# factoryofthesun/distraytracer

Hardware: AMD Instinct MI355X
Metric: Mpixel-samples/s (W×H×spp/s) + wall-clock per frame, 1/2/4/8 GPU (higher is better)
Workload: dtype f64; 1 GPU; buildFinal(240) 1920x1080, 64 spp, depth 8, brdf_samples 2, DoF aperture 0.2, glossy + Cook-Torrance + 4 area lights; use_model=0, frame=240, xRes=1920, yRes=1080, spp=64, max_depth=8, parallelism=single GPU, 2 frame(s) in flight

## Files before the change

distraytracer_amd/__init__.py:

```python
import ctypes

from ._lib import (DATA_DIR, DT_KERNEL_AUTO, DT_KERNEL_DONATE, DT_KERNEL_PRODUCT, DT_OUT_IMAGE, DT_OUT_SLAB, AccelInfo, BVHNode, Camera, DenoiseParams, DenoiseVarParams, DTError, Globals, SceneDesc,
                   SHAPE_TYPES, OcclusionParams, RayOrderParams, DT_RAY_ORDER_TILE, Stats, TemporalParams, Tiles, UpsampleParams, check, lib)

__all__ = ["Globals", "Tiles", "Stats", "DTError", "globals_default", "build_scene", "Scene",
           "render", "render_sky", "renderImage", "renderImageCloud", "write_ppm", "DATA_DIR",
           "DT_OUT_IMAGE", "DT_OUT_SLAB", "slab_floats", "slab_floats_max", "unpack_slabs", "tiles", "check", "lib",
           "accel_info", "DT_KERNEL_AUTO", "DT_KERNEL_PRODUCT", "DT_KERNEL_DONATE",
           "accum_doubles", "window_check", "render_window", "render_window_async", "resolve", "Progressive",
           "mean_abs_change", "adapt_converged", "render_window_adaptive", "resolve_adaptive", "adapt_select_ms",
           "AdaptiveProgressive", "render_features", "feature_images", "FEATURE_PLANES",
           "DenoiseParams", "denoise_params_default", "denoise", "denoised_filename",
           "DenoiseVarParams", "denoise_var_params_default", "variance",
           "Camera", "camera", "TemporalParams", "temporal_params_default", "reproject", "TemporalAccumulator",
           "trace_rays", "rays_occluded", "RAY_PLANES",
           "trace_rays_multi", "segment_through_glass", "RAY_MULTI_PLANES",
           "rays_transmittance", "RAY_TRANSMIT_PLANES",
           "camera_rays", "camera_rays_rows", "rays_resolve", "peel_layers", "RESOLVE_MODES",
           "RayOrderParams", "RayOrder", "ray_order_params_default", "ray_order_key", "ray_order", "DT_RAY_ORDER_TILE",
           "render_mattes", "matte_mask", "shape_groups", "MATTE_PLANES",
           "UpsampleParams", "upsample_params_default", "upsample", "low_res_globals",
           "OcclusionParams", "occlusion_params_default", "render_occlusion", "occlusion_ao_ray", "occlusion_light_ray",
           "occlusion_images", "points_occlusion", "shape_texels", "bake_occlusion"]


def globals_default():
    g = Globals()
    lib.dt_globals_default(ctypes.byref(g))
    return g


# ... 8 lines not shown

    @property
    def desc(self):
        return self._ptr.contents

    def __del__(self):
        if getattr(self, "_ptr", None) and lib is not None:
            lib.dt_scene_desc_free(self._ptr)
            self._ptr = None


def build_scene(name, frame, g, data_dir=DATA_DIR):
    out = ctypes.POINTER(SceneDesc)()
    check(lib.dt_build_scene(name.encode(), float(frame), ctypes.byref(g), data_dir.encode(), ctypes.byref(out)),
          "dt_build_scene(%s)" % name)
    return BuiltScene(out)


def accel_info(built, g):
    info = AccelInfo()
    desc = built._ptr if isinstance(built, BuiltScene) else ctypes.pointer(built)
    check(lib.dt_accel_info_build(desc, ctypes.byref(g), ctypes.byref(info)), "dt_accel_info_build")
    return info.as_dict()


def trace_build(built, g, frame):
    name = ctypes.create_string_buffer(64)
    sf, bf = ctypes.c_uint32(), ctypes.c_uint32()
    desc = built._ptr if isinstance(built, BuiltScene) else ctypes.pointer(built)
    check(lib.dt_trace_build(desc, ctypes.byref(g), int(frame), name, 64, ctypes.byref(sf), ctypes.byref(bf)),
          "dt_trace_build")
    return name.value.decode(), sf.value, bf.value


class Scene:

    def __init__(self, built, g, upload=True):
        self._h = ctypes.c_void_p()
        desc = built._ptr if isinstance(built, BuiltScene) else ctypes.pointer(built)
        self._keep = built
        if upload:
            check(lib.dt_scene_create(desc, ctypes.byref(g), ctypes.byref(self._h)), "dt_scene_create")
        else:
            check(lib.dt_scene_prepare(desc, ctypes.byref(g), ctypes.byref(self._h)), "dt_scene_prepare")

    def upload(self):
# ... 1548 lines not shown
```

distraytracer_amd/_lib.py:

```python
import ctypes
import os

_HERE = os.path.dirname(os.path.abspath(__file__))
LIB_PATH = os.environ.get("DT_LIB") or os.path.join(_HERE, "libdt.so")
REPO_ROOT = os.path.dirname(_HERE)
DATA_DIR = os.path.join(REPO_ROOT, "data")

c_int32, c_uint32, c_int64, c_uint64 = ctypes.c_int32, ctypes.c_uint32, ctypes.c_int64, ctypes.c_uint64
c_float, c_double = ctypes.c_float, ctypes.c_double
D3 = c_double * 3

DT_OK = 0
DT_OUT_IMAGE = 0
DT_OUT_SLAB = 1
DT_KERNEL_AUTO, DT_KERNEL_PRODUCT, DT_KERNEL_DONATE = 0, 1, 2

SHAPE_TYPES = {1: "sphere", 2: "cylinder", 3: "triangle", 4: "rectangle", 5: "rectprism_v2",
               6: "checkerboard", 7: "checkerboard_hole", 8: "checker_cylinder", 9: "rectprism_cyl"}
ABI_VERSION = 8


class ShapeDesc(ctypes.Structure):
    _fields_ = [("type", c_int32), ("model", c_int32), ("material", c_int32), ("emit", c_int32),
                ("flags", c_uint32), ("tex_frame", c_int32), ("roughness", c_float), ("radius", c_float),
# ... 146 lines not shown

class History(ctypes.Structure):
    _fields_ = [("colour", ctypes.c_void_p), ("var", ctypes.c_void_p), ("len", ctypes.c_void_p)]


class BVHNode(ctypes.Structure):
    _fields_ = [("first_child", c_int32), ("n_children", c_int32), ("first_index", c_int32),
                ("n_indices", c_int32), ("leaf", c_int32), ("depth", c_int32), ("lbound", D3), ("ubound", D3)]


class AccelInfo(ctypes.Structure):
    _fields_ = [("n_nodes", c_int32), ("n_fnodes", c_int32), ("n_bnodes", c_int32), ("boxes_ordered", c_int32),
                ("sg_lights", c_int32), ("sg_dim", c_int32 * 3), ("sg_cells", c_int64), ("sg_tree_cells", c_int64),
                ("sg_list_pool", c_int64), ("sg_list_entries", c_int64), ("nodes_hash", c_uint64),
                ("fnodes_hash", c_uint64), ("bnodes_hash", c_uint64), ("sg_hash", c_uint64),
                ("sg_contents_hash", c_uint64), ("bump_pad", c_float), ("sg_reach", c_float),
                ("sg_umbra_cells", c_int64), ("features", ctypes.c_uint32),
                ("sg_sub_blocks", c_int32), ("sg_sub_nodes", c_int64), ("sg_sub_hash", c_uint64)]

    def as_dict(self):
        d = {k: getattr(self, k) for k, _ in self._fields_}
        d["sg_dim"] = tuple(self.sg_dim)
        return d


EXPORTS = ["dt_abi_version", "dt_last_error", "dt_globals_default", "dt_scene_create", "dt_scene_destroy",
           "dt_scene_prepare", "dt_scene_upload", "dt_scene_set_kernel",
           "dt_scene_bvh", "dt_bvh_build", "dt_accel_info_build", "dt_trace_build", "dt_slab_floats", "dt_slab_floats_max",
           "dt_render", "dt_render_async", "dt_collect_stats", "dt_debug_counters", "dt_debug_item_costs", "dt_render_sky",
           "dt_unpack_slabs", "dt_build_scene", "dt_scene_desc_free", "dt_write_ppm", "dt_write_png",
           "dt_mocap_bone_table", "dt_debug_normalize", "dt_debug_vdiv", "dt_debug_vnorm", "dt_debug_light_edges",
           "dt_intersect_primary",
           "dt_debug_load_obj",
           "dt_accum_doubles", "dt_window_check", "dt_render_window", "dt_render_window_async", "dt_resolve",
           "dt_adapt_converged", "dt_render_window_adaptive", "dt_render_window_adaptive_async",
           "dt_resolve_adaptive", "dt_adapt_select_ms", "dt_render_features",
           "dt_denoise_params_default", "dt_denoise_workspace_floats", "dt_denoise",
           "dt_variance", "dt_denoise_var_params_default", "dt_denoise_var_workspace_floats", "dt_denoise_var",
           "dt_camera_get", "dt_temporal_params_default", "dt_reproject",
           "dt_trace_rays", "dt_rays_occluded", "dt_render_mattes", "dt_matte_mask",
           "dt_upsample_params_default", "dt_upsample",
           "dt_guide_bounce", "dt_render_features_path",
           "dt_occlusion_params_default", "dt_render_occlusion", "dt_occlusion_ao_ray", "dt_occlusion_light_ray",
           "dt_points_occlusion",
           "dt_ray_order_params_default", "dt_ray_order_key", "dt_ray_order_workspace_bytes", "dt_ray_order",
           "dt_permute_rows",
           "dt_trace_rays_multi",
           "dt_camera_rays_rows", "dt_camera_rays", "dt_rays_resolve",
           "dt_rays_transmittance", "dt_points_occlusion_glass"]


class DTError(RuntimeError):
    pass


def _share_torch_hip_runtime():
    try:
        import torch
    except ImportError:
        pass


def _load():
    _share_torch_hip_runtime()
    if not os.path.exists(LIB_PATH):
        raise DTError("libdt.so not built (%s): run __graft_entry__.build() / make -C "
                      "distraytracer_amd/csrc" % LIB_PATH)
    lib = ctypes.CDLL(LIB_PATH)
    lib.dt_abi_version.restype = c_int32
    if lib.dt_abi_version() != ABI_VERSION:
        raise DTError("libdt.so ABI %d, this binding expects %d: rebuild (make -C distraytracer_amd/csrc)"
                      % (lib.dt_abi_version(), ABI_VERSION))
    P = ctypes.POINTER
    sig = {
        "dt_abi_version": (c_int32, []),
        "dt_last_error": (ctypes.c_char_p, []),
        "dt_globals_default": (None, [P(Globals)]),
        "dt_scene_create": (c_int32, [P(SceneDesc), P(Globals), P(ctypes.c_void_p)]),
        "dt_scene_destroy": (None, [ctypes.c_void_p]),
        "dt_scene_prepare": (c_int32, [P(SceneDesc), P(Globals), P(ctypes.c_void_p)]),
        "dt_scene_upload": (c_int32, [ctypes.c_void_p]),
        "dt_scene_set_kernel": (c_int32, [ctypes.c_void_p, c_int32]),
        "dt_scene_bvh": (c_int32, [ctypes.c_void_p, P(BVHNode), c_int32, P(c_int32), c_int32, P(c_int32),
                                   P(c_int32)]),
        "dt_bvh_build": (c_int32, [P(SceneDesc), P(Globals), P(BVHNode), c_int32, P(c_int32), c_int32, P(c_int32),
                                   P(c_int32)]),
        "dt_accel_info_build": (c_int32, [P(SceneDesc), P(Globals), P(AccelInfo)]),
        "dt_trace_build": (c_int32, [P(SceneDesc), P(Globals), c_int32, ctypes.c_char_p, c_int32,
                                     P(ctypes.c_uint32), P(ctypes.c_uint32)]),
        "dt_slab_floats": (c_int64, [P(Globals), P(Tiles)]),
        "dt_slab_floats_max": (c_int64, [P(Globals), P(Tiles)]),
        "dt_render": (c_int32, [ctypes.c_void_p, P(Globals), c_int32, P(Tiles), ctypes.c_void_p, c_int32,
                                ctypes.c_void_p, P(Stats)]),
        "dt_render_async": (c_int32, [ctypes.c_void_p, P(Globals), c_int32, P(Tiles), ctypes.c_void_p,
                                      ctypes.c_void_p]),
        "dt_collect_stats": (c_int32, [ctypes.c_void_p, ctypes.c_void_p, P(Stats)]),
        "dt_accum_doubles": (c_int64, [P(Globals), P(Tiles)]),
        "dt_window_check": (c_int32, [P(Globals), c_int32, c_int32]),
        "dt_render_window": (c_int32, [ctypes.c_void_p, P(Globals), c_int32, P(Tiles), c_int32, c_int32,
                                       ctypes.c_void_p, ctypes.c_void_p, P(Stats)]),
        "dt_render_window_async": (c_int32, [ctypes.c_void_p, P(Globals), c_int32, P(Tiles), c_int32, c_int32,
                                             ctypes.c_void_p, ctypes.c_void_p]),
        "dt_resolve": (c_int32, [P(Globals), P(Tiles), ctypes.c_void_p, c_int32, ctypes.c_void_p, c_int32,
                                 ctypes.c_void_p, P(c_uint64)]),
        "dt_adapt_converged": (c_int32, [P(c_double), P(c_double), ctypes.c_uint32, c_double, c_int32]),
        "dt_render_window_adaptive": (c_int32, [ctypes.c_void_p, P(Globals), c_int32, P(Tiles), c_int32, c_int32,
                                                ctypes.c_void_p, ctypes.c_void_p, ctypes.c_void_p, c_double, c_int32,
                                                ctypes.c_void_p, P(Stats)]),
        "dt_render_window_adaptive_async": (c_int32, [ctypes.c_void_p, P(Globals), c_int32, P(Tiles), c_int32, c_int32,
                                                      ctypes.c_void_p, ctypes.c_void_p, ctypes.c_void_p, c_double,
# ... 104 lines not shown
```

distraytracer_amd/csrc/dt_api.cpp:

```cpp
#include <hip/hip_runtime.h>
#include <zlib.h>

#include <chrono>
#include <cmath>
#include <cstdio>
#include <cstdlib>
#include <cstring>
#include <algorithm>
#include <string>
#include <vector>

#include "dt_adapt.h"
#include "dt_guide.h"
#include "dt_occl.h"
#include "host_internal.h"
#include "host_launch.h"

using namespace dth;

extern "C" size_t dt_launch_size(void);
extern "C" size_t dt_scene_struct_offset(void);
extern "C" size_t dt_scene_struct_size(void);
extern "C" size_t dt_params_struct_offset(void);
extern "C" hipError_t dt_launch_sky(const void* dev_launch, float* out, int64_t n_threads, hipStream_t stream);
// ... 560 lines not shown
    auto mix = [&](uint64_t x) { h = (h ^ x) * 1099511628211ull; };
    for (uint32_t x : a.sg.sub_blocks) mix(x);
    info->sg_sub_hash = (h ^ nodes_hash(a.sg.sub_nodes)) * 1099511628211ull;
  }
  info->sg_lights = a.sg.n_lights;
  for (int k = 0; k < 3; ++k) info->sg_dim[k] = a.sg.dim[k];
  info->sg_cells = (int64_t)(a.sg.cells.size() / 2);
  for (size_t c = 0; c + 1 < a.sg.cells.size(); c += 2) {
    if (a.sg.cells[c + 1] == DT_SG_WALK) info->sg_tree_cells++;
    else info->sg_list_entries += a.sg.cells[c + 1];
  }
  info->sg_list_pool = (int64_t)a.sg.list.size();
  info->nodes_hash = nodes_hash(a.dnodes);
  info->fnodes_hash = a.n_fnodes ? nodes_hash(a.fnodes) : 0;
  info->bnodes_hash = a.n_bnodes ? nodes_hash(a.bnodes) : 0;
  info->sg_hash = sg_hash(a.sg, false);
  info->sg_contents_hash = sg_hash(a.sg, true);
  info->bump_pad = a.bump_pad;
  info->sg_reach = a.sg.reach;
  info->sg_umbra_cells = a.sg.umbra_cells;
  return DT_OK;
}

int64_t dt_slab_floats(const dt_globals* g, const dt_tiles* tiles)
{
  dtd::DParams P;
  std::string err;
  if (!g || fill_sky_params(*g, 0.0f, tiles, P, err)) return -1;
  return P.n_owned_tiles * P.tw * P.th * 3;
}

int64_t dt_slab_floats_max(const dt_globals* g, const dt_tiles* tiles)
{
  if (!g || !tiles) return -1;
  dt_tiles t = *tiles;
  t.rank = 0;
  return dt_slab_floats(g, &t);
}

static int prepare_render(const dt_scene* sc, const dt_globals* g, int32_t frame, const dt_tiles* tiles,
                          dtd::DParams& P, std::vector<float>& zs)
{
  std::string err;
  int rc = fill_params(*g, frame, tiles, P, err);
  if (rc) return fail(rc, err);
  const int need = g->max_depth * (2 + (g->brdf_samples > 1 ? g->brdf_samples : 1));
// ... 1762 lines not shown
```

distraytracer_amd/csrc/host_accel.cpp:

```cpp
#include <algorithm>
#include <cmath>
#include <cstdio>
#include <cstdlib>
#include <cstring>

#include "host_internal.h"

namespace dth {

bool sg_parse_block(const char* s, int& bx, int& by)
{
  bx = 8;
  by = 4;
  if (!s) return true;
  if (strcmp(s, "0") == 0) {
    bx = by = 1;
    return true;
  }
  int x = 0, y = 0;
  char tail = 0;
  if (sscanf(s, "%dx%d%c", &x, &y, &tail) == 2 && x >= 1 && y >= 1) {
    bx = x;
    by = y;
    return true;
// ... 43 lines not shown
  {
    const char* bt = getenv("DT_BUMP_TREE");
    const double d = fabs((double)g.frame_range) * (1.0 + 1e-3) + 1e-3;
    const char* bps = getenv("DT_BUMP_PAD_SCALE");
    const double pad = (((double)fabsf(g.move_per_frame) * d + (double)fabsf(g.accel_t) * d * d * d) * 1.01 + 1e-6) *
                       (bps ? atof(bps) : 1.0);
    a.bump_pad = (float)pad;

    if (!(bt && bt[0] == '0') && g.blur_samples > 0 && pad > 0 && pad < 1e3 && build_fast_tree(dnodes, a.bnodes, pad, eye, up_only))
      a.n_bnodes = (int)a.bnodes.size();
    else
      a.bnodes.clear();
  }
  if (a.bnodes.empty()) a.bnodes.push_back(dnodes.empty() ? dtd::DNodeDev() : dnodes[0]);
  if (a.bparent.empty()) a.bparent.push_back(-1);
  stage("bump tree");
  for (const dtd::DShapeHdr& h : f.hdr)
    if (h.type == DT_SHAPE_RECTPRISM_CYL) a.no_cull = true;
  const char* sgv = getenv("DT_SHADOW_GRID");
  const char* sgc = getenv("DT_SG_CELLS");
  const char* sgr = getenv("DT_SG_REACH");
  const char* sgs = getenv("DT_SG_START");
  const int start_mode = sgs ? atoi(sgs) : 1;
  const double ypad_main = a.n_bnodes > 0 ? (double)a.bump_pad : 0.0;
  if ((sgv && sgv[0] == '0') || a.no_cull ||
      !build_shadow_grid(dnodes, f, a.sg, sgc ? atof(sgc) : 32768.0, sgr ? (float)atof(sgr) : DT_SG_REACH_DEFAULT,
                         ypad_main, up_only, start_mode == 2 ? g.eye : nullptr, (double)g.aperture))
    a.sg = ShadowGrid();
  else if (start_mode == 1) {
    size_t walk = 0, cells = a.sg.cells.size() / 2;
    for (size_t c = 0; c < cells; ++c) walk += a.sg.cells[2 * c + 1] == DT_SG_WALK;
    ShadowGrid s2;
    if (walk <= cells / 10 &&
        build_shadow_grid(dnodes, f, s2, sgc ? atof(sgc) : 32768.0, sgr ? (float)atof(sgr) : DT_SG_REACH_DEFAULT,
                          ypad_main, up_only, g.eye, (double)g.aperture))
      a.sg = std::move(s2);
  }
  for (int l = 0; l < DT_MAX_SGRID; ++l) a.sg.base0[l] = a.sg.base[l];
  if (a.sg.ypad > 0 && !a.sg.cells.empty()) {
    size_t walk = 0, cells = a.sg.cells.size() / 2;
    for (size_t c = 0; c < cells; ++c) walk += a.sg.cells[2 * c + 1] == DT_SG_WALK;
    const char* p0 = getenv("DT_SG_PASS0");
    const bool want = p0 ? p0[0] == '1' : walk > cells / 10;
    ShadowGrid g0;
    if (want && build_shadow_grid(dnodes, f, g0, sgc ? atof(sgc) : 32768.0, sgr ? (float)atof(sgr) : DT_SG_REACH_DEFAULT, 0.0) &&
        g0.n_lights == a.sg.n_lights && g0.dim[0] == a.sg.dim[0] && g0.dim[1] == a.sg.dim[1] && g0.dim[2] == a.sg.dim[2]) {
      const uint32_t cell_off = (uint32_t)(a.sg.cells.size() / 2), list_off = (uint32_t)a.sg.list.size();
      for (size_t c = 0; c < g0.cells.size(); c += 2) {
        uint32_t o = g0.cells[c];
        if (g0.cells[c + 1] != DT_SG_WALK) o = (o & DT_SG_UMBRA) | ((o & ~DT_SG_UMBRA) + list_off);
        a.sg.cells.push_back(o);
        a.sg.cells.push_back(g0.cells[c + 1]);
      }
      a.sg.list.insert(a.sg.list.end(), g0.list.begin(), g0.list.end());
      for (int l = 0; l < DT_MAX_SGRID; ++l) a.sg.base0[l] = g0.base[l] >= 0 ? g0.base[l] + (int32_t)cell_off : -1;
      a.sg.umbra_cells += g0.umbra_cells;
    }
  }
// ... 51 lines not shown
```

distraytracer_amd/csrc/host_internal.h:

```cpp
#pragma once
#include <cstdint>
#include <functional>
#include <string>
#include <array>
#include <vector>

#include "../../include/dt.h"
#include "dt_math.h"
#include "dt_scene_dev.h"

namespace dth {

struct FlatBVH {
  std::vector<dtd::DNode> nodes;
  std::vector<int32_t> leaf_idx;
  std::vector<int32_t> depth;
  std::vector<int32_t> n_children;
};

void shape_bounds(const dt_shape_desc& sh, dtm::V3& lb, dtm::V3& ub);
void build_bvh(const dt_scene_desc& d, const dt_globals& g, FlatBVH& out);
bool build_fast_tree(const std::vector<dtd::DNodeDev>& ref, std::vector<dtd::DNodeDev>& out, double ypad = 0,
                     const double* eye = nullptr, bool up_only = false);
void build_fast_subtree(const std::vector<dtd::DNodeDev>& ref, const std::vector<int32_t>& leaf_nodes,
// ... 28 lines not shown
inline P3 sub3(const P3& a, const P3& b) { return {a[0] - b[0], a[1] - b[1], a[2] - b[2]}; }
inline P3 mad3(const P3& a, const P3& b, double s) { return {a[0] + s * b[0], a[1] + s * b[1], a[2] + s * b[2]}; }
bool shape_hull_points(const dtd::DShapeHdr& h, const double* g, double ypad, std::vector<P3>& pts,
                       bool up_only = false);
bool leaf_hull_points(const FlatScene& fs, const dtd::DNodeDev& leaf, int skip_shape, double ypad, std::vector<P3>& out,
                      bool up_only = false);
double hull_gap(const P3* A, int na, const P3* B, int nb, const P3& v);
bool hulls_separated(const P3* A, int na, const P3* B, int nb, double margin, P3& hint);

inline void blur_leaf_pad(const dtd::DNodeDev& n, double ypad, bool up_only, double& below, double& above)
{
  below = above = ypad;
  if (!up_only || !(n.meta & dtd::DN_SINGLE)) return;
  const int type = (int)((n.meta >> 4) & 15u);
  const uint32_t flags = (n.meta >> 8) & 0xffu;
  if (type == DT_SHAPE_TRIANGLE || type == DT_SHAPE_RECTANGLE || type == DT_SHAPE_RECTPRISM_V2 ||
      type == DT_SHAPE_CHECKERBOARD || type == DT_SHAPE_CHECKERBOARD_HOLE) {
    below = 0;
    above = (flags & DT_F_NAMED_RECT) ? ypad : 0;
  }
}
bool build_shadow_grid(const std::vector<dtd::DNodeDev>& nodes, const FlatScene& fs, ShadowGrid& g,
                       double target_cells = 32768, float reach = 0.5f, double ypad = 0, bool up_only = false,
                       const double* cam = nullptr, double cam_r = 0);

struct FlatScene {
  FlatBVH bvh;
  std::vector<dtd::DShapeHdr> hdr;
  std::vector<double> geom;
  std::vector<dtd::DMat> mat;
  std::vector<dtd::DLight> lights;
  std::vector<uint8_t> tex;
};
int flatten_scene(const dt_scene_desc& d, const dt_globals& g, FlatScene& out, std::string& err);

bool sg_parse_block(const char* s, int& bx, int& by);

struct Accel {
  std::vector<dtd::DNodeDev> dnodes;
  std::vector<dtd::DNodeDev> fnodes;
  std::vector<dtd::DNodeDev> bnodes;
  std::vector<int32_t> bparent;
  std::vector<int32_t> leaf;
  int n_fnodes = 0, n_bnodes = 0;
  float bump_pad = 0;
  bool bump_up_only = false;
  bool no_cull = false;
// ... 26 lines not shown
```

distraytracer_amd/csrc/host_shadowgrid.cpp:

```cpp
#include <algorithm>
#include <array>
#include <atomic>
#include <chrono>
#include <cstdio>
#include <cstdlib>
#include <cmath>
#include <thread>
#include <vector>

#include "host_internal.h"

namespace dth {

namespace {

bool segment_meets_box(const double p[3], const double q[3], const double lo[3], const double hi[3])
{
  double t0 = 0.0, t1 = 1.0;
  for (int a = 0; a < 3; ++a) {
    const double d = q[a] - p[a];
    if (std::fabs(d) < 1e-300) {
      if (p[a] < lo[a] || p[a] > hi[a]) return false;
      continue;
    }
// ... 95 lines not shown
        for (int a = 0; a < 3; ++a)
          cen[a] += (R[dtd::R_A + a] + 0.5 * (R[dtd::R_V1N + a] * R[dtd::R_LEN1] + R[dtd::R_V2N + a] * R[dtd::R_LEN2])) / 6;
      }
      for (int f = 0; f < 6; ++f) {
        const double* R = g + dtd::PR_F + f * dtd::R_SIZE;
        const double* A = R + dtd::R_A;
        const double* n = R + dtd::R_N;
        const double nn = std::sqrt(n[0] * n[0] + n[1] * n[1] + n[2] * n[2]);
        if (!(nn > 0)) continue;
        const double side = ((cen[0] - A[0]) * n[0] + (cen[1] - A[1]) * n[1] + (cen[2] - A[2]) * n[2]) / nn;
        if (!(std::fabs(side) > 1e-6)) continue;
        if (!plane_range(A, n, clo, chi, llo, lhi, mn, mx)) continue;
        if ((side > 0 && mx < -m) || (side < 0 && mn > m)) return true;
      }
      return false;
    }
  }
  return false;
}

}

bool build_shadow_grid(const std::vector<dtd::DNodeDev>& nodes, const FlatScene& fs, ShadowGrid& g,
                       double target_cells, float reach, double ypad, bool up_only, const double* cam, double cam_r)
{
  const double t_entry = std::chrono::duration<double, std::milli>(std::chrono::steady_clock::now().time_since_epoch()).count();
  const std::vector<dtd::DLight>& lights = fs.lights;
  g = ShadowGrid();
  for (int l = 0; l < DT_MAX_SGRID; ++l) g.sub_base[l] = -1;
  g.reach = reach;
  g.ypad = ypad;
  if (nodes.empty() || !(nodes[0].lb[0] <= nodes[0].ub[0])) return false;
  std::vector<int> leaves;
  for (size_t i = 0; i < nodes.size(); ++i)
    if (nodes[i].meta & dtd::DN_LEAF) leaves.push_back((int)i);
  const char* ml = getenv("DT_SG_MAX_LEAVES");
  if (leaves.empty() || leaves.size() > (ml ? (size_t)atol(ml) : (size_t)4096)) return false;
  std::vector<double> leaf_hi[3];
  {
    std::vector<P3> pts;
    auto shape_hi = [&](int sid, double hi[3]) {
      const dtd::DShapeHdr& hd = fs.hdr[sid];
      const double* gp = fs.geom.data() + hd.off;
      if (hd.type == DT_SHAPE_SPHERE) {
        const double r = std::sqrt(gp[dtd::SP_R2]);
        for (int a = 0; a < 3; ++a) hi[a] = gp[dtd::SP_C + a] + r;
      } else if (hd.type == DT_SHAPE_CYLINDER || hd.type == DT_SHAPE_CHECKER_CYLINDER) {
// ... 80 lines not shown
  const double m1 = (reach + 0.05) * hmax_ + slack;
  const double m2 = 2e-3 + slack;
  const double mplane = 1e-3 + 1e-6 * (1 + scale);
  std::vector<std::array<double, 6>> lbox(nodes.size());
  for (int leaf : leaves) {
    double below = 0, above = 0;
    if (ypad > 0) blur_leaf_pad(nodes[leaf], ypad, up_only, below, above);
    for (int a = 0; a < 3; ++a) {
      lbox[leaf][a] = nodes[leaf].lb[a] - (a == 1 ? below : 0.0);
      lbox[leaf][3 + a] = nodes[leaf].ub[a] + (a == 1 ? above : 0.0);
    }
  }
  auto leaf_shapes = [&](int leaf, std::vector<int>& out) {
    out.clear();
    const dtd::DNodeDev& nd = nodes[leaf];
    if (nd.meta & dtd::DN_SINGLE) out.push_back(nd.first);
    else
      for (int64_t q = 0; q < (int64_t)nd.aux; ++q) out.push_back(fs.bvh.leaf_idx[nd.first + q]);
  };
  long dropped = 0;
  std::atomic<long> start_dropped(0);
  const bool timing = getenv("DT_TIMING") != nullptr;
  const bool start_on = cam != nullptr;
  const size_t nshape = fs.hdr.size();
  const int ncell_all = g.dim[0] * g.dim[1] * g.dim[2];
  constexpr int NK = 4;
  const double eta_k[NK] = {1.25e-7, 2e-3, 1e-6, 1e-6};
  std::vector<int32_t> occ3, bocc3;
  std::vector<double> occ;
  std::vector<int8_t> s_plane;
  struct SPlane {
    double n[3], c, maxd, move;
    double dblo, dbhi;
    double mvs[2];
    double sD[DT_MAX_SGRID];
    double box[6];
  };
  std::vector<SPlane> sp;
  const int OB = 8, OB2 = 4;
  int ob_nx = 0, ob_ny = 0;
  std::vector<double> bocc;
  if (start_on) {
    double olo[3], ohi[3];
    for (int a = 0; a < 3; ++a) {
      olo[a] = std::min((double)nodes[0].lb[a], cam[a] - cam_r);
      ohi[a] = std::max((double)nodes[0].ub[a], cam[a] + cam_r);
    }
    double diag = 0;
    for (int a = 0; a < 3; ++a) diag += (ohi[a] - olo[a]) * (ohi[a] - olo[a]);
    diag = std::sqrt(diag) * 1.02;
    occ.assign((size_t)ncell_all * 6 * NK, 0.0);
    for (size_t c = 0; c < (size_t)ncell_all * NK; ++c)
      for (int a = 0; a < 3; ++a) { occ[c * 6 + a] = INFINITY; occ[c * 6 + 3 + a] = -INFINITY; }
    ob_nx = (g.dim[0] + OB - 1) / OB;
    ob_ny = (g.dim[1] + OB2 - 1) / OB2;
    bocc.assign((size_t)ob_nx * ob_ny * g.dim[2] * 6 * NK, 0.0);
    for (size_t c = 0; c < bocc.size() / 6; ++c)
      for (int a = 0; a < 3; ++a) { bocc[c * 6 + a] = INFINITY; bocc[c * 6 + 3 + a] = -INFINITY; }
    struct SBox { double lo[3], hi[3], pad; int k, sid; bool refl, glossy; };
    std::vector<SBox> sbox;
    bool bounded = true;
    std::vector<P3> pts;
    for (size_t sid = 0; sid < nshape && bounded; ++sid) {
      const dtd::DShapeHdr& hd = fs.hdr[sid];
      const double* gp = fs.geom.data() + hd.off;
      SBox b;
      double* blo = b.lo;
      double* bhi = b.hi;
      int k = 1;
      const int mt = fs.mat[sid].material;
      b.refl = mt == DT_MAT_GLASS || mt == DT_MAT_STEEL || mt == DT_MAT_ALUMINUM || mt == DT_MAT_WATER ||
               mt == DT_MAT_LINOLEUM;
      b.glossy = (fs.mat[sid].flags & DT_F_GLOSSY) != 0;
      pts.clear();
      if (hd.type == DT_SHAPE_SPHERE) {
        const double r = std::sqrt(gp[dtd::SP_R2]);
        for (int a = 0; a < 3; ++a) { blo[a] = gp[dtd::SP_C + a] - r; bhi[a] = gp[dtd::SP_C + a] + r; }
      } else if (hd.type == DT_SHAPE_CYLINDER || hd.type == DT_SHAPE_CHECKER_CYLINDER) {
        const double r = std::sqrt(gp[dtd::CY_R2]);
        for (int a = 0; a < 3; ++a) {
          blo[a] = std::min(gp[dtd::CY_C1 + a], gp[dtd::CY_C2 + a]) - r;
          bhi[a] = std::max(gp[dtd::CY_C1 + a], gp[dtd::CY_C2 + a]) + r;
        }
      } else if (shape_hull_points(hd, gp, 0.0, pts) && !pts.empty()) {
        k = 2;
        for (int a = 0; a < 3; ++a) { blo[a] = INFINITY; bhi[a] = -INFINITY; }
        for (const P3& q : pts)
          for (int a = 0; a < 3; ++a) { blo[a] = std::min(blo[a], q[a]); bhi[a] = std::max(bhi[a], q[a]); }
// ... 147 lines not shown
          double d = -P.c;
          for (int a = 0; a < 3; ++a) d += P.n[a] * (((q >> a) & 1) ? ohi[a] : olo[a]);
          md = std::max(md, std::fabs(d));
        }
        P.move = (ypad > 0 && hd.type == DT_SHAPE_RECTANGLE && (hd.flags & DT_F_NAMED_RECT))
                     ? std::fabs(P.n[1]) * ypad * (1 + 1e-9) + 1e-12 : 0.0;
        P.maxd = 1.02 * md + 1e-3 + P.move;
        for (int sd = 0; sd < 2; ++sd)
          P.mvs[sd] = P.move == 0.0 || !up_only ? P.move
                                                : std::max(0.0, (sd ? 1.0 : -1.0) * P.n[1]) * ypad * (1 + 1e-9) + 1e-12;
        P.dblo = INFINITY;
        P.dbhi = -INFINITY;
        for (int q = 0; q < 8; ++q) {
          double d = -P.c;
          for (int a = 0; a < 3; ++a) d += P.n[a] * (((q >> a) & 1) ? g.org_hi[a] : g.org_lo[a]);
          P.dblo = std::min(P.dblo, d);
          P.dbhi = std::max(P.dbhi, d);
        }
        s_plane[sid] = 1;
        int zeros = 0;
        for (int a = 0; a < 3; ++a) zeros += P.n[a] == 0.0;
        if (zeros < 2) {
          s_plane[sid] = 2;
          for (int a = 0; a < 3; ++a) { P.box[a] = sbox[sid].lo[a]; P.box[3 + a] = sbox[sid].hi[a]; }
        }
      }
    }
  }
  auto start_separated = [&](int sid, size_t l, const double* clo, const double* chi, const int* c0, const int* c1,
                             const double* llo, const double* lhi) {
    if (occ.empty() || !s_plane[sid]) return false;
    const SPlane& P = sp[sid];
    const double sD = P.sD[l];
    if (sD == 0) return false;
    const double s = sD > 0 ? 1.0 : -1.0, D = std::fabs(sD);
    const bool one = c0[0] == c1[0] && c0[1] == c1[1] && c0[2] == c1[2];
    int32_t id3 = -1;
    if (one) {
      id3 = occ3[((size_t)c0[2] * g.dim[1] + c0[1]) * g.dim[0] + c0[0]];
    } else {
      for (int z = c0[2]; z <= c1[2]; ++z)
        for (int by = c0[1] / OB2; by <= c1[1] / OB2; ++by)
          for (int bx = c0[0] / OB; bx <= c1[0] / OB; ++bx) {
            const int32_t q3 = bocc3[((size_t)z * ob_ny + by) * ob_nx + bx];
            if (q3 != -1) id3 = id3 == -1 || id3 == q3 ? q3 : -2;
          }
    }
    if (s_plane[sid] == 2 && id3 != sid) {
      const double* b = P.box;
      if (b[0] <= chi[0] && b[3] >= clo[0] && b[1] <= chi[1] && b[4] >= clo[1] && b[2] <= chi[2] && b[5] >= clo[2])
        return false;
    }
    const double* n = P.n;
    const double c = P.c, mv = P.mvs[sD > 0 ? 1 : 0];
    double lmax2 = 0, lmin2 = 0;
    for (int a = 0; a < 3; ++a) {
      const double far = std::max(std::fabs(chi[a] - llo[a]), std::fabs(lhi[a] - clo[a]));
      const double gap = std::max({0.0, llo[a] - chi[a], clo[a] - lhi[a]});
      lmax2 += far * far;
      lmin2 += gap * gap;
    }
    if (!(lmin2 > 4e-6)) return false;
    double mn = INFINITY;
    for (int k = 0; k < NK; ++k) {
      if (k == 3 && id3 == sid) {
        const double dmax = std::max(std::fabs(P.dblo), std::fabs(P.dbhi)) + P.move;
        mn = std::min(mn, -1.25e-7 * dmax * (1 + 1e-6) - 1e-12 * (1 + scale));
        continue;
      }
      double blo[3] = {INFINITY, INFINITY, INFINITY}, bhi[3] = {-INFINITY, -INFINITY, -INFINITY};
      auto take = [&](const double* o) {
        for (int a = 0; a < 3; ++a) { blo[a] = std::min(blo[a], o[a]); bhi[a] = std::max(bhi[a], o[3 + a]); }
      };
      if (one) {
        take(occ.data() + (((size_t)c0[2] * g.dim[1] + c0[1]) * g.dim[0] + c0[0]) * 6 * NK + k * 6);
      } else {
        for (int z = c0[2]; z <= c1[2]; ++z)
          for (int by = c0[1] / OB2; by <= c1[1] / OB2; ++by)
            for (int bx = c0[0] / OB; bx <= c1[0] / OB; ++bx)
              take(bocc.data() + (((size_t)z * ob_ny + by) * ob_nx + bx) * 6 * NK + k * 6);
      }
      if (!(blo[0] <= bhi[0] && blo[1] <= bhi[1] && blo[2] <= bhi[2])) continue;
      double d = -s * c, ulo = -c, uhi = -c;
      for (int a = 0; a < 3; ++a) {
        d += std::min(s * n[a] * blo[a], s * n[a] * bhi[a]);
        ulo += std::min(n[a] * blo[a], n[a] * bhi[a]);
        uhi += std::max(n[a] * blo[a], n[a] * bhi[a]);
      }
      const double span = std::max(uhi, P.dbhi) - std::min(ulo, P.dblo);
      mn = std::min(mn, d - mv - eta_k[k] * span * (1 + 1e-6) - 1e-12 * (1 + scale));
    }
    const double d_o = std::min(mn, 0.0) + 1e-3 * D / std::sqrt(lmax2);
    return d_o > 1e-7 * (1 + scale);
  };
  const char* so = getenv("DT_SG_ORDER");
  const bool order_lists = so && atoi(so) != 0;
  const char* sh = getenv("DT_SG_HULL");
  const int hull_cull = sh ? atoi(sh) : 1;
  const char* sq = getenv("DT_SG_QUAD");
  const bool quad_hull = !(sq && sq[0] == '0');
  const char* mls = getenv("DT_SG_MAX_LIST");
  const int max_list = mls && atoi(mls) > 0 ? atoi(mls) : DT_SGRID_MAX_LIST;
  int blk_x = 8, blk_y = 4;
  if (!sg_parse_block(getenv("DT_SG_BLOCK"), blk_x, blk_y))
    fprintf(stderr, "dt: DT_SG_BLOCK='%s' not understood (use 0 or XxY with X, Y >= 1): default 8x4\n",
            getenv("DT_SG_BLOCK"));
  auto now_ms = [] { return std::chrono::duration<double, std::milli>(std::chrono::steady_clock::now().time_since_epoch()).count(); };
  const int hw_threads = (int)std::max(1u, std::thread::hardware_concurrency());

  const char* su = getenv("DT_SG_UMBRA");
  const bool umbra_on = !(su && su[0] == '0');
  const bool umbra_cells_too = su && su[0] == '2';
  const double mu = m2 + mplane;
  struct Face { P3 A, n, v1, v2; double c, len1, len2; };
  std::vector<Face> faces_all;
  std::vector<int> face_shape;
// ... 115 lines not shown
    if (L.type == DT_LIGHT_POINT) S.lhull.push_back({L.center[0], L.center[1], L.center[2]});
    else
      for (int k = 1; k < 5; ++k) S.lhull.push_back({S.lpts[k][0], S.lpts[k][1], S.lpts[k][2]});
    if (!umbra_on) continue;
    double lmax = 0;
    for (int k = 0; k < 8; ++k) {
      const P3 p = {lo[0] + ((k & 1) ? ext[0] : 0), lo[1] + ((k & 2) ? ext[1] : 0), lo[2] + ((k & 4) ? ext[2] : 0)};
      for (const P3& q : S.lhull) lmax = std::max(lmax, std::sqrt(dot3(sub3(p, q), sub3(p, q))));
    }
    S.mud = std::max(mu, 2e-3 * (lmax + 1));
    for (size_t fi = 0; fi < faces_all.size(); ++fi) {
      if (face_shape[fi] == L.shape_index) continue;
      const Face& f = faces_all[fi];
      double qmn = INFINITY, qmx = -INFINITY;
      for (const P3& q : S.lhull) {
        const double d = dot3(f.n, q) - f.c;
        qmn = std::min(qmn, d);
        qmx = std::max(qmx, d);
      }
      if (qmn > S.mud || qmx < -S.mud) S.fl.push_back((int)fi);
    }
  }
  if (!occ.empty()) {
    for (size_t sid = 0; sid < nshape; ++sid) {
      if (!s_plane[sid]) continue;
      SPlane& P = sp[sid];
      for (size_t l = 0; l < nl; ++l) {
        P.sD[l] = 0;
        if (!ls[l].on) continue;
        double dlo = INFINITY, dhi = -INFINITY;
        for (int q = 0; q < 8; ++q) {
          double d = -P.c;
          for (int a = 0; a < 3; ++a) d += P.n[a] * (((q >> a) & 1) ? ls[l].lhi[a] : ls[l].llo[a]);
          dlo = std::min(dlo, d);
          dhi = std::max(dhi, d);
        }
        const int side = dlo > 0 ? 1 : dhi < 0 ? -1 : 0;
        const double D = (side > 0 ? dlo : -dhi) - (side > 0 ? P.mvs[1] : P.mvs[0]);
        if (side != 0 && D - 1e-3 > 1e-5 * P.maxd) P.sD[l] = side * D;
      }
    }
  }
  const int UBX = std::max(1, blk_x), UBY = std::max(1, blk_y);
  const int unby = (g.dim[1] + UBY - 1) / UBY, unrows = unby * g.dim[2];
  auto umbra_rows = [&](size_t l, std::vector<int32_t>& um, int t, int nt) {
    const LightSetup& S = ls[l];
    for (int row = t; row < unrows; row += nt) {
      const int z = row / unby, yb = (row % unby) * UBY, ye = std::min(yb + UBY, g.dim[1]) - 1;
      for (int xb = 0; xb < g.dim[0]; xb += UBX) {
        const int xe = std::min(xb + UBX, g.dim[0]) - 1;
        double clo[3], chi[3];
        const int c0[3] = {xb, yb, z}, c1[3] = {xe, ye, z};
        for (int a = 0; a < 3; ++a) {
          clo[a] = lo[a] + c0[a] * hh[a] - m1;
          chi[a] = lo[a] + (c1[a] + 1) * hh[a] + m1;
        }
        for (int fi : S.fl) {
          const Face& f = faces_all[fi];
          const int32_t leaf = shape_leaf[face_shape[fi]];
          const int r = box_umbra(f, clo, chi, S.lhull, S.mud);
          if (r < 0) continue;
          if (r == 0 && !umbra_cells_too) continue;
          if (r > 0) {
            for (int y = yb; y <= ye; ++y)
// ... 399 lines not shown
```

include/dt.h:

```cpp
#ifndef DT_H
#define DT_H

#include <stdint.h>

#ifdef __cplusplus
extern "C" {
#endif

#define DT_ABI_VERSION 8

#define DT_OK              0
#define DT_E_INVALID      -1
#define DT_E_NO_DEVICE    -2
#define DT_E_OOM          -3
#define DT_E_UNSUPPORTED  -4
#define DT_E_IO           -5
#define DT_E_LIMIT        -6

enum dt_shape_type {
  DT_SHAPE_SPHERE           = 1,
  DT_SHAPE_CYLINDER         = 2,
  DT_SHAPE_TRIANGLE         = 3,
  DT_SHAPE_RECTANGLE        = 4,
  DT_SHAPE_RECTPRISM_V2     = 5,
// ... 176 lines not shown
} dt_bvh_node;
int  dt_scene_bvh(const dt_scene* s, dt_bvh_node* nodes, int32_t cap,
                  int32_t* indices, int32_t index_cap, int32_t* n_nodes, int32_t* n_indices);

int  dt_bvh_build(const dt_scene_desc* desc, const dt_globals* g, dt_bvh_node* nodes, int32_t cap,
                  int32_t* indices, int32_t index_cap, int32_t* n_nodes, int32_t* n_indices);

typedef struct dt_accel_info {
  int32_t n_nodes, n_fnodes, n_bnodes, boxes_ordered;
  int32_t sg_lights, sg_dim[3];
  int64_t sg_cells, sg_tree_cells, sg_list_pool, sg_list_entries;
  uint64_t nodes_hash, fnodes_hash, bnodes_hash;
  uint64_t sg_hash;
  uint64_t sg_contents_hash;
  float bump_pad, sg_reach;
  int64_t sg_umbra_cells;
  uint32_t features;
  int32_t sg_sub_blocks;
  int64_t sg_sub_nodes;
  uint64_t sg_sub_hash;
} dt_accel_info;
int dt_accel_info_build(const dt_scene_desc* desc, const dt_globals* g, dt_accel_info* info);

int dt_trace_build(const dt_scene_desc* desc, const dt_globals* g, int32_t frame, char* name, int32_t name_cap,
                   uint32_t* scene_features, uint32_t* build_features);

int64_t dt_slab_floats(const dt_globals* g, const dt_tiles* tiles);
int64_t dt_slab_floats_max(const dt_globals* g, const dt_tiles* tiles);

int dt_render(const dt_scene* s, const dt_globals* g, int32_t frame, const dt_tiles* tiles,
              float* out, int32_t out_on_device, void* stream, dt_stats* stats);
int dt_render_async(const dt_scene* s, const dt_globals* g, int32_t frame, const dt_tiles* tiles,
                    float* out_device, void* stream);
int dt_collect_stats(const dt_scene* s, void* stream, dt_stats* stats);

int64_t dt_accum_doubles(const dt_globals* g, const dt_tiles* tiles);
int dt_window_check(const dt_globals* g, int32_t begin, int32_t end);
int dt_render_window(const dt_scene* s, const dt_globals* g, int32_t frame, const dt_tiles* tiles,
                     int32_t begin, int32_t end, double* accum_device, void* stream, dt_stats* stats);
int dt_render_window_async(const dt_scene* s, const dt_globals* g, int32_t frame, const dt_tiles* tiles,
                           int32_t begin, int32_t end, double* accum_device, void* stream);
int dt_resolve(const dt_globals* g, const dt_tiles* tiles, const double* accum, int32_t n_samples,
               float* out, int32_t on_device, void* stream, uint64_t* nan_pixels);

int dt_adapt_converged(const double s1[3], const double s2[3], uint32_t count, double tol, int32_t min_samples);
int dt_render_window_adaptive(const dt_scene* s, const dt_globals* g, int32_t frame, const dt_tiles* tiles,
// ... 269 lines not shown
```

Measured before the change: 4469 Mpixel-samples/s.

## Use rectangular-prism faces as start-side separating planes in shadow grid culling

Extends the shadow-grid build so each axis-aligned face of a rectangular prism can act as a separating plane when deciding whether a shape can block light from a grid cell. Each face gets a conservative slack bound derived from the other faces. This lets more shapes be dropped from per-cell shadow candidate lists, which means fewer shadow-ray intersection tests on the GPU. It adds host-side build cost and relies on the conservative bounds being correct. The change also adds an introspection API that exports the per-cell shadow lists.

```diff
diff --git a/distraytracer_amd/__init__.py b/distraytracer_amd/__init__.py
--- a/distraytracer_amd/__init__.py
+++ b/distraytracer_amd/__init__.py
@@ -6,7 +6,7 @@
 __all__ = ["Globals", "Tiles", "Stats", "DTError", "globals_default", "build_scene", "Scene",
            "render", "render_sky", "renderImage", "renderImageCloud", "write_ppm", "DATA_DIR",
            "DT_OUT_IMAGE", "DT_OUT_SLAB", "slab_floats", "slab_floats_max", "unpack_slabs", "tiles", "check", "lib",
-           "accel_info", "DT_KERNEL_AUTO", "DT_KERNEL_PRODUCT", "DT_KERNEL_DONATE",
+           "accel_info", "accel_sg_lists", "DT_KERNEL_AUTO", "DT_KERNEL_PRODUCT", "DT_KERNEL_DONATE",
            "accum_doubles", "window_check", "render_window", "render_window_async", "resolve", "Progressive",
            "mean_abs_change", "adapt_converged", "render_window_adaptive", "resolve_adaptive", "adapt_select_ms",
            "AdaptiveProgressive", "render_features", "feature_images", "FEATURE_PLANES",
@@ -61,6 +61,21 @@
     desc = built._ptr if isinstance(built, BuiltScene) else ctypes.pointer(built)
     check(lib.dt_accel_info_build(desc, ctypes.byref(g), ctypes.byref(info)), "dt_accel_info_build")
     return info.as_dict()
+
+
+def accel_sg_lists(built, g):
+    import numpy as np
+    from ._lib import SGGrid
+    desc = built._ptr if isinstance(built, BuiltScene) else ctypes.pointer(built)
+    grid, n = SGGrid(), ctypes.c_int64(0)
+    check(lib.dt_accel_sg_lists(desc, ctypes.byref(g), ctypes.byref(grid), None, 0, ctypes.byref(n)),
+          "dt_accel_sg_lists")
+    ent = np.zeros((n.value, 3), dtype=np.int32)
+    check(lib.dt_accel_sg_lists(desc, ctypes.byref(g), ctypes.byref(grid), ent.ctypes.data, n.value, ctypes.byref(n)),
+          "dt_accel_sg_lists")
+    info = {"n_lights": grid.n_lights, "dim": tuple(grid.dim), "lo": tuple(grid.lo), "inv_h": tuple(grid.inv_h),
+            "reach": grid.reach, "base": tuple(grid.base), "n_records": grid.n_records}
+    return info, ent
 
 
 def trace_build(built, g, frame):
diff --git a/distraytracer_amd/_lib.py b/distraytracer_amd/_lib.py
--- a/distraytracer_amd/_lib.py
+++ b/distraytracer_amd/_lib.py
@@ -192,6 +192,11 @@
         d = {k: getattr(self, k) for k, _ in self._fields_}
         d["sg_dim"] = tuple(self.sg_dim)
         return d
+
+
+class SGGrid(ctypes.Structure):
+    _fields_ = [("n_lights", c_int32), ("dim", c_int32 * 3), ("lo", c_float * 3), ("inv_h", c_float * 3),
+                ("reach", c_float), ("base", c_int32 * 16), ("n_records", c_int64)]
 
 
 EXPORTS = ["dt_abi_version", "dt_last_error", "dt_globals_default", "dt_scene_create", "dt_scene_destroy",
@@ -217,7 +222,8 @@
            "dt_permute_rows",
            "dt_trace_rays_multi",
            "dt_camera_rays_rows", "dt_camera_rays", "dt_rays_resolve",
-           "dt_rays_transmittance", "dt_points_occlusion_glass"]
+           "dt_rays_transmittance", "dt_points_occlusion_glass",
+           "dt_accel_sg_lists"]
 
 
 class DTError(RuntimeError):
@@ -256,6 +262,7 @@
         "dt_bvh_build": (c_int32, [P(SceneDesc), P(Globals), P(BVHNode), c_int32, P(c_int32), c_int32, P(c_int32),
                                    P(c_int32)]),
         "dt_accel_info_build": (c_int32, [P(SceneDesc), P(Globals), P(AccelInfo)]),
+        "dt_accel_sg_lists": (c_int32, [P(SceneDesc), P(Globals), P(SGGrid), ctypes.c_void_p, c_int64, P(c_int64)]),
         "dt_trace_build": (c_int32, [P(SceneDesc), P(Globals), c_int32, ctypes.c_char_p, c_int32,
                                      P(ctypes.c_uint32), P(ctypes.c_uint32)]),
         "dt_slab_floats": (c_int64, [P(Globals), P(Tiles)]),
diff --git a/distraytracer_amd/csrc/dt_api.cpp b/distraytracer_amd/csrc/dt_api.cpp
--- a/distraytracer_amd/csrc/dt_api.cpp
+++ b/distraytracer_amd/csrc/dt_api.cpp
@@ -606,6 +606,52 @@
   return DT_OK;
 }
 
+int dt_accel_sg_lists(const dt_scene_desc* desc, const dt_globals* g, dt_sg_grid* grid, int32_t* entries, int64_t cap,
+                      int64_t* n_entries)
+{
+  if (!desc || !g || !grid || !n_entries) return fail(DT_E_INVALID, "null argument");
+  if (desc->n_shapes < 0 || (desc->n_shapes > 0 && !desc->shapes)) return fail(DT_E_INVALID, "invalid descriptor");
+  FlatScene f;
+  std::string err;
+  int rc = flatten_scene(*desc, *g, f, err);
+  if (rc) return fail(rc, err);
+  Accel a;
+  build_accel(f, *g, a);
+  memset(grid, 0, sizeof(*grid));
+  grid->n_lights = a.sg.n_lights;
+  grid->reach = a.sg.reach;
+  for (int k = 0; k < 3; ++k) {
+    grid->dim[k] = a.sg.dim[k];
+    grid->lo[k] = a.sg.lo[k];
+    grid->inv_h[k] = a.sg.inv_h[k];
+  }
+  for (int l = 0; l < DT_MAX_SGRID; ++l) grid->base[l] = l < a.sg.n_lights ? a.sg.base[l] : -1;
+  grid->n_records = (int64_t)(a.sg.cells.size() / 2);
+  int64_t n = 0;
+  auto put = [&](int64_t rec, int32_t leaf, int32_t shape) {
+    if (entries && n < cap) {
+      entries[3 * n] = (int32_t)rec;
+      entries[3 * n + 1] = leaf;
+      entries[3 * n + 2] = shape;
+    }
+    ++n;
+  };
+  for (size_t c = 0; c + 1 < a.sg.cells.size(); c += 2) {
+    const int64_t rec = (int64_t)(c / 2);
+    if (a.sg.cells[c + 1] == DT_SG_WALK) { put(rec, -1, -1); continue; }
+    const uint32_t off = a.sg.cells[c] & ~DT_SG_UMBRA;
+    for (uint32_t k = 0; k < a.sg.cells[c + 1]; ++k) {
+      const int32_t leaf = a.sg.list[off + k];
+      const dtd::DNodeDev& nd = a.dnodes[(size_t)leaf];
+      if (nd.meta & dtd::DN_SINGLE) put(rec, leaf, (int32_t)nd.first);
+      else
+        for (int64_t q = 0; q < (int64_t)nd.aux; ++q) put(rec, leaf, f.bvh.leaf_idx[nd.first + q]);
+    }
+  }
+  *n_entries = n;
+  return DT_OK;
+}
+
 int64_t dt_slab_floats(const dt_globals* g, const dt_tiles* tiles)
 {
   dtd::DParams P;
diff --git a/distraytracer_amd/csrc/host_accel.cpp b/distraytracer_amd/csrc/host_accel.cpp
--- a/distraytracer_amd/csrc/host_accel.cpp
+++ b/distraytracer_amd/csrc/host_accel.cpp
@@ -89,10 +89,12 @@
   const char* sgr = getenv("DT_SG_REACH");
   const char* sgs = getenv("DT_SG_START");
   const int start_mode = sgs ? atoi(sgs) : 1;
+  const char* sgp = getenv("DT_SG_START_PRISM");
+  const bool start_prism = !(sgp && sgp[0] == '0');
   const double ypad_main = a.n_bnodes > 0 ? (double)a.bump_pad : 0.0;
   if ((sgv && sgv[0] == '0') || a.no_cull ||
       !build_shadow_grid(dnodes, f, a.sg, sgc ? atof(sgc) : 32768.0, sgr ? (float)atof(sgr) : DT_SG_REACH_DEFAULT,
-                         ypad_main, up_only, start_mode == 2 ? g.eye : nullptr, (double)g.aperture))
+                         ypad_main, up_only, start_mode == 2 ? g.eye : nullptr, (double)g.aperture, start_prism))
     a.sg = ShadowGrid();
   else if (start_mode == 1) {
     size_t walk = 0, cells = a.sg.cells.size() / 2;
@@ -100,7 +102,7 @@
     ShadowGrid s2;
     if (walk <= cells / 10 &&
         build_shadow_grid(dnodes, f, s2, sgc ? atof(sgc) : 32768.0, sgr ? (float)atof(sgr) : DT_SG_REACH_DEFAULT,
-                          ypad_main, up_only, g.eye, (double)g.aperture))
+                          ypad_main, up_only, g.eye, (double)g.aperture, start_prism))
       a.sg = std::move(s2);
   }
   for (int l = 0; l < DT_MAX_SGRID; ++l) a.sg.base0[l] = a.sg.base[l];
diff --git a/distraytracer_amd/csrc/host_internal.h b/distraytracer_amd/csrc/host_internal.h
--- a/distraytracer_amd/csrc/host_internal.h
+++ b/distraytracer_amd/csrc/host_internal.h
@@ -74,7 +74,7 @@
 }
 bool build_shadow_grid(const std::vector<dtd::DNodeDev>& nodes, const FlatScene& fs, ShadowGrid& g,
                        double target_cells = 32768, float reach = 0.5f, double ypad = 0, bool up_only = false,
-                       const double* cam = nullptr, double cam_r = 0);
+                       const double* cam = nullptr, double cam_r = 0, bool start_prism = true);
 
 struct FlatScene {
   FlatBVH bvh;
diff --git a/distraytracer_amd/csrc/host_shadowgrid.cpp b/distraytracer_amd/csrc/host_shadowgrid.cpp
--- a/distraytracer_amd/csrc/host_shadowgrid.cpp
+++ b/distraytracer_amd/csrc/host_shadowgrid.cpp
@@ -141,7 +141,8 @@
 }
 
 bool build_shadow_grid(const std::vector<dtd::DNodeDev>& nodes, const FlatScene& fs, ShadowGrid& g,
-                       double target_cells, float reach, double ypad, bool up_only, const double* cam, double cam_r)
+                       double target_cells, float reach, double ypad, bool up_only, const double* cam, double cam_r,
+                       bool start_prism)
 {
   const double t_entry = std::chrono::duration<double, std::milli>(std::chrono::steady_clock::now().time_since_epoch()).count();
   const std::vector<dtd::DLight>& lights = fs.lights;
@@ -268,6 +269,7 @@
   std::atomic<long> start_dropped(0);
   const bool timing = getenv("DT_TIMING") != nullptr;
   const bool start_on = cam != nullptr;
+  const bool prism_on = start_on && start_prism;
   const size_t nshape = fs.hdr.size();
   const int ncell_all = g.dim[0] * g.dim[1] * g.dim[2];
   constexpr int NK = 4;
@@ -281,8 +283,12 @@
     double mvs[2];
     double sD[DT_MAX_SGRID];
     double box[6];
+    double slack = 0;
+    int out = 0;
   };
   std::vector<SPlane> sp;
+  std::vector<SPlane> spp;
+  std::vector<int32_t> pr_first, pr_n;
   const int OB = 8, OB2 = 4;
   int ob_nx = 0, ob_ny = 0;
   std::vector<double> bocc;
@@ -305,11 +311,45 @@
       for (int a = 0; a < 3; ++a) { bocc[c * 6 + a] = INFINITY; bocc[c * 6 + 3 + a] = -INFINITY; }
     struct SBox { double lo[3], hi[3], pad; int k, sid; bool refl, glossy; };
     std::vector<SBox> sbox;
+    std::vector<int> sbox_first(nshape, -1);
     bool bounded = true;
     std::vector<P3> pts;
     for (size_t sid = 0; sid < nshape && bounded; ++sid) {
       const dtd::DShapeHdr& hd = fs.hdr[sid];
       const double* gp = fs.geom.data() + hd.off;
+      sbox_first[sid] = (int)sbox.size();
+      if (prism_on && hd.type == DT_SHAPE_RECTPRISM_V2) {
+        for (int f = 0; f < 6; ++f) {
+          const double* R = gp + dtd::PR_F + f * dtd::R_SIZE;
+          SBox b;
+          for (int a = 0; a < 3; ++a) { b.lo[a] = INFINITY; b.hi[a] = -INFINITY; }
+          for (int q = 0; q < 4; ++q)
+            for (int a = 0; a < 3; ++a) {
+              const double p = R[dtd::R_A + a] + ((q & 1) ? R[dtd::R_V1N + a] * R[dtd::R_LEN1] : 0.0) +
+                               ((q & 2) ? R[dtd::R_V2N + a] * R[dtd::R_LEN2] : 0.0);
+              b.lo[a] = std::min(b.lo[a], p);
+              b.hi[a] = std::max(b.hi[a], p);
+            }
+          double sd = 0;
+          for (int a = 0; a < 3; ++a) sd += (b.hi[a] - b.lo[a]) * (b.hi[a] - b.lo[a]);
+          if (!std::isfinite(sd)) { bounded = false; break; }
+          const double rho = 1e-6 * (1 + std::sqrt(sd));
+          int flat = -1;
+          for (int a = 0; a < 3; ++a)
+            if (b.hi[a] == b.lo[a] && R[dtd::R_N + (a + 1) % 3] == 0.0 && R[dtd::R_N + (a + 2) % 3] == 0.0) flat = a;
+          for (int a = 0; a < 3; ++a)
+            if (a != flat) { b.lo[a] -= rho; b.hi[a] += rho; }
+          const int mt = fs.mat[sid].material;
+          b.refl = mt == DT_MAT_GLASS || mt == DT_MAT_STEEL || mt == DT_MAT_ALUMINUM || mt == DT_MAT_WATER ||
+                   mt == DT_MAT_LINOLEUM;
+          b.glossy = (fs.mat[sid].flags & DT_F_GLOSSY) != 0;
+          b.pad = 0;
+          b.k = 2;
+          b.sid = (int)sid;
+          sbox.push_back(b);
+        }
+        continue;
+      }
       SBox b;
       double* blo = b.lo;
       double* bhi = b.hi;
@@ -503,15 +543,126 @@
         for (int a = 0; a < 3; ++a) zeros += P.n[a] == 0.0;
         if (zeros < 2) {
           s_plane[sid] = 2;
-          for (int a = 0; a < 3; ++a) { P.box[a] = sbox[sid].lo[a]; P.box[3 + a] = sbox[sid].hi[a]; }
-        }
-      }
-    }
-  }
-  auto start_separated = [&](int sid, size_t l, const double* clo, const double* chi, const int* c0, const int* c1,
-                             const double* llo, const double* lhi) {
-    if (occ.empty() || !s_plane[sid]) return false;
-    const SPlane& P = sp[sid];
+          const SBox& own = sbox[(size_t)sbox_first[sid]];
+          for (int a = 0; a < 3; ++a) { P.box[a] = own.lo[a]; P.box[3 + a] = own.hi[a]; }
+        }
+      }
+    }
+    if (!occ.empty() && prism_on) {
+      pr_first.assign(nshape, -1);
+      pr_n.assign(nshape, 0);
+      double wlo[3], whi[3];
+      for (int a = 0; a < 3; ++a) { wlo[a] = olo[a]; whi[a] = ohi[a]; }
+      for (const dtd::DLight& L : lights)
+        for (int a = 0; a < 3; ++a) {
+          const double q[5] = {L.center[a], L.A[a], L.B[a], L.D[a], L.B[a] + L.D[a] - L.A[a]};
+          for (int k = 0; k < (L.type == DT_LIGHT_RECT ? 5 : 1); ++k) {
+            wlo[a] = std::min(wlo[a], q[k] - 3e-3);
+            whi[a] = std::max(whi[a], q[k] + 3e-3);
+          }
+        }
+      double Rb = 0, cmax = 0;
+      for (int a = 0; a < 3; ++a) {
+        Rb += (whi[a] - wlo[a]) * (whi[a] - wlo[a]);
+        cmax = std::max({cmax, std::fabs(wlo[a]), std::fabs(whi[a])});
+      }
+      Rb = std::sqrt(Rb) * 1.02 + 1;
+      const double sigma = 1e-14 * (1 + Rb + cmax);
+      const double u23 = 0x1p-23, ortho = 1e-12;
+      for (size_t sid = 0; sid < nshape; ++sid) {
+        const dtd::DShapeHdr& hd = fs.hdr[sid];
+        if (hd.type != DT_SHAPE_RECTPRISM_V2) continue;
+        const double* gp = fs.geom.data() + hd.off;
+        double cen[3] = {0, 0, 0};
+        for (int f = 0; f < 6; ++f) {
+          const double* R = gp + dtd::PR_F + f * dtd::R_SIZE;
+          for (int a = 0; a < 3; ++a)
+            cen[a] += (R[dtd::R_A + a] + 0.5 * (R[dtd::R_V1N + a] * R[dtd::R_LEN1] + R[dtd::R_V2N + a] * R[dtd::R_LEN2])) / 6;
+        }
+        for (int f = 0; f < 6; ++f) {
+          const double* R = gp + dtd::PR_F + f * dtd::R_SIZE;
+          const double* n = R + dtd::R_N;
+          const double nn = std::sqrt(n[0] * n[0] + n[1] * n[1] + n[2] * n[2]);
+          if (!(nn > 0) || !std::isfinite(nn)) continue;
+          if ((n[0] == 0.0) + (n[1] == 0.0) + (n[2] == 0.0) != 2) continue;
+          SPlane P;
+          for (int a = 0; a < 3; ++a) P.n[a] = n[a] / nn;
+          P.c = P.n[0] * R[dtd::R_A] + P.n[1] * R[dtd::R_A + 1] + P.n[2] * R[dtd::R_A + 2];
+          const double dcen = P.n[0] * cen[0] + P.n[1] * cen[1] + P.n[2] * cen[2] - P.c;
+          if (!(std::fabs(dcen) > 1e-6)) continue;
+          P.out = dcen < 0 ? 1 : -1;
+          double U = 0;
+          for (int f2 = 0; f2 < 6; ++f2) {
+            if (f2 == f) continue;
+            const double* G = gp + dtd::PR_F + f2 * dtd::R_SIZE;
+            const double* A = G + dtd::R_A;
+            const double* v[2] = {G + dtd::R_V1N, G + dtd::R_V2N};
+            const double len[2] = {G[dtd::R_LEN1], G[dtd::R_LEN2]};
+            const double dA = P.out * (P.n[0] * A[0] + P.n[1] * A[1] + P.n[2] * A[2] - P.c);
+            double UG = INFINITY;
+            bool edge = false;
+            for (int k = 0; k < 2; ++k) {
+              const double nv = P.out * (P.n[0] * v[k][0] + P.n[1] * v[k][1] + P.n[2] * v[k][2]);
+              const double s = nv >= 0 ? 1.0 : -1.0;
+              double r2 = 0;
+              for (int a = 0; a < 3; ++a) r2 += (P.out * P.n[a] - s * v[k][a]) * (P.out * P.n[a] - s * v[k][a]);
+              const double rr = std::sqrt(r2);
+              if (!(rr <= 1e-6) || !(len[k] >= 0)) continue;
+              UG = std::min(UG, dA + (s > 0 ? len[k] * (1 + u23) : 0.0) + sigma + rr * Rb);
+              edge = true;
+            }
+            {
+              const double* gn = G + dtd::R_N;
+              const double gnn = std::sqrt(gn[0] * gn[0] + gn[1] * gn[1] + gn[2] * gn[2]);
+              auto dt3 = [](const double* x, const double* y) { return x[0] * y[0] + x[1] * y[1] + x[2] * y[2]; };
+              const bool frame_ok = gnn > 0 && std::isfinite(gnn) && std::fabs(dt3(v[0], v[1])) <= ortho &&
+                                    std::fabs(dt3(v[0], gn)) <= ortho * gnn && std::fabs(dt3(v[1], gn)) <= ortho * gnn &&
+                                    std::fabs(dt3(v[0], v[0]) - 1) <= ortho && std::fabs(dt3(v[1], v[1]) - 1) <= ortho &&
+                                    len[0] >= 0 && len[1] >= 0;
+              if (frame_ok) {
+                double cm = dA, s12 = 0;
+                for (int k = 0; k < 2; ++k) {
+                  const double nv = P.out * dt3(P.n, v[k]);
+                  cm += std::max(0.0, len[k] * nv);
+                  s12 += std::fabs(nv);
+                }
+                const double off = eta_k[2] * Rb;
+                const double sg = sigma + off + u23 * std::max(len[0], len[1]) + 8 * ortho * Rb;
+                UG = std::min(UG, cm + s12 * sg + off);
+              }
+            }
+            if (!edge && !(UG <= 0)) UG = INFINITY;
+            U = std::max(U, UG);
+          }
+          if (!(8 * U < 1e-3)) continue;
+          P.slack = U;
+          P.move = 0;
+          P.mvs[0] = P.mvs[1] = 0;
+          double md = 0;
+          P.dblo = INFINITY;
+          P.dbhi = -INFINITY;
+          for (int q = 0; q < 8; ++q) {
+            double d = -P.c, e = -P.c;
+            for (int a = 0; a < 3; ++a) {
+              d += P.n[a] * (((q >> a) & 1) ? ohi[a] : olo[a]);
+              e += P.n[a] * (((q >> a) & 1) ? g.org_hi[a] : g.org_lo[a]);
+            }
+            md = std::max(md, std::fabs(d));
+            P.dblo = std::min(P.dblo, e);
+            P.dbhi = std::max(P.dbhi, e);
+          }
+          P.maxd = 1.02 * md + 1e-3;
+          if (pr_n[sid] == 0) pr_first[sid] = (int32_t)spp.size();
+          ++pr_n[sid];
+          spp.push_back(P);
+          s_plane[sid] = 3;
+        }
+      }
+      if (timing) fprintf(stderr, "dt: start-side prism faces tried as culled planes: %zu\n", spp.size());
+    }
+  }
+  auto plane_start_separated = [&](const SPlane& P, int kind, int sid, size_t l, const double* clo, const double* chi,
+                                   const int* c0, const int* c1, const double* llo, const double* lhi) {
     const double sD = P.sD[l];
     if (sD == 0) return false;
     const double s = sD > 0 ? 1.0 : -1.0, D = std::fabs(sD);
@@ -527,7 +678,7 @@
             if (q3 != -1) id3 = id3 == -1 || id3 == q3 ? q3 : -2;
           }
     }
-    if (s_plane[sid] == 2 && id3 != sid) {
+    if (kind == 2 && id3 != sid) {
       const double* b = P.box;
       if (b[0] <= chi[0] && b[3] >= clo[0] && b[1] <= chi[1] && b[4] >= clo[1] && b[2] <= chi[2] && b[5] >= clo[2])
         return false;
@@ -572,7 +723,15 @@
       mn = std::min(mn, d - mv - eta_k[k] * span * (1 + 1e-6) - 1e-12 * (1 + scale));
     }
     const double d_o = std::min(mn, 0.0) + 1e-3 * D / std::sqrt(lmax2);
-    return d_o > 1e-7 * (1 + scale);
+    return d_o > 1e-7 * (1 + scale) + 8 * P.slack;
+  };
+  auto start_separated = [&](int sid, size_t l, const double* clo, const double* chi, const int* c0, const int* c1,
+                             const double* llo, const double* lhi) {
+    if (occ.empty() || !s_plane[sid]) return false;
+    if (s_plane[sid] != 3) return plane_start_separated(sp[sid], s_plane[sid], sid, l, clo, chi, c0, c1, llo, lhi);
+    for (int32_t q = 0; q < pr_n[sid]; ++q)
+      if (plane_start_separated(spp[(size_t)pr_first[sid] + q], 3, sid, l, clo, chi, c0, c1, llo, lhi)) return true;
+    return false;
   };
   const char* so = getenv("DT_SG_ORDER");
   const bool order_lists = so && atoi(so) != 0;
@@ -734,12 +893,11 @@
     }
   }
   if (!occ.empty()) {
-    for (size_t sid = 0; sid < nshape; ++sid) {
-      if (!s_plane[sid]) continue;
-      SPlane& P = sp[sid];
+    auto light_sides = [&](SPlane& P) {
       for (size_t l = 0; l < nl; ++l) {
         P.sD[l] = 0;
         if (!ls[l].on) continue;
+        if (P.out != 0 && lights[l].type != DT_LIGHT_RECT) continue;
         double dlo = INFINITY, dhi = -INFINITY;
         for (int q = 0; q < 8; ++q) {
           double d = -P.c;
@@ -749,9 +907,12 @@
         }
         const int side = dlo > 0 ? 1 : dhi < 0 ? -1 : 0;
         const double D = (side > 0 ? dlo : -dhi) - (side > 0 ? P.mvs[1] : P.mvs[0]);
-        if (side != 0 && D - 1e-3 > 1e-5 * P.maxd) P.sD[l] = side * D;
-      }
-    }
+        if (side != 0 && (P.out == 0 || side == P.out) && D - 1e-3 > 1e-5 * P.maxd + 8 * P.slack) P.sD[l] = side * D;
+      }
+    };
+    for (size_t sid = 0; sid < nshape; ++sid)
+      if (s_plane[sid] == 1 || s_plane[sid] == 2) light_sides(sp[sid]);
+    for (SPlane& P : spp) light_sides(P);
   }
   const int UBX = std::max(1, blk_x), UBY = std::max(1, blk_y);
   const int unby = (g.dim[1] + UBY - 1) / UBY, unrows = unby * g.dim[2];
diff --git a/include/dt.h b/include/dt.h
--- a/include/dt.h
+++ b/include/dt.h
@@ -222,6 +222,15 @@
 } dt_accel_info;
 int dt_accel_info_build(const dt_scene_desc* desc, const dt_globals* g, dt_accel_info* info);
 
+typedef struct dt_sg_grid {
+  int32_t n_lights, dim[3];
+  float   lo[3], inv_h[3], reach;
+  int32_t base[16];
+  int64_t n_records;
+} dt_sg_grid;
+int dt_accel_sg_lists(const dt_scene_desc* desc, const dt_globals* g, dt_sg_grid* grid, int32_t* entries,
+                      int64_t cap, int64_t* n_entries);
+
 int dt_trace_build(const dt_scene_desc* desc, const dt_globals* g, int32_t frame, char* name, int32_t name_cap,
                    uint32_t* scene_features, uint32_t* build_features);
 
```

Result: no change. 4492 Mpixel-samples/s, median of 6 (+0.5%).
